# uzh-rpg/EvDeblurNeRF

Hardware: AMD Instinct MI355X
Metric: rays/sec (4096x128 samples, 8x256 MLP) (higher is better)
Workload: dtype f16c (compensated f16: one f16 MFMA product + two block-scaled fp6 MFMA products of the operands' rounding residuals; f32 accumulate; ~2^-15 operands); 1 GPU; nerf8x256 render: 4096 rays x 128 samples per GPU, PE(10,4)+MLP+composite, ndc, viewdirs; rays_per_gpu=4096, samples=128, precision=f16c

## Files before the change

evdeblurnerf_amd/csrc/evd_api.hip:

```cpp
#include <atomic>
#include "evd_common.h"
#include "nerf_mlp.h"
#include "nerf_mlp_kernel.h"
#include "nerf_net.h"
#include "nerf_train.h"
#include "pack.h"

#include <cmath>
#include <cstdint>
#include <cstdlib>
#include <cstring>
#include <vector>

namespace evd {

char* err_buf() {
    static thread_local char buf[512] = {0};
    return buf;
}

int fail(int code, const char* fmt, ...) {
    va_list ap;
    va_start(ap, fmt);
    vsnprintf(err_buf(), 512, fmt, ap);
    va_end(ap);
    return code;
}

int nerf_mlp_generic_dispatch(int prec, int W, const MlpParams& p, hipStream_t st);
int nerf_mlp_pipe_dispatch(int prec, const MlpParams& p, hipStream_t st);
int nerf_mlp_c_dispatch(int W, int D, int skip, const MlpParams& p, hipStream_t st);
int nerf_mlp_c_chunks(int W, int D, int skip, bool train);

static __global__ void k_fold_feature(const float* __restrict__ views_w, const float* __restrict__ views_b, const float* __restrict__ feature_w,
                                      const float* __restrict__ feature_b, int W, int ICV, float* __restrict__ wfold, float* __restrict__ bfold) {
    const int in = W + ICV, rows = W / 2;
    const long i = (long)blockIdx.x * 256 + threadIdx.x;
    if (i < (long)rows * in) {
        const int r = (int)(i / in), c = (int)(i % in);
        if (c >= W) { wfold[i] = views_w[i]; return; }
        double acc = 0.0;
        for (int k = 0; k < W; ++k) acc = fma((double)views_w[(long)r * in + k], (double)feature_w[(long)k * W + c], acc);
        wfold[i] = (float)acc;
    } else if (i < (long)rows * in + rows) {
        const int r = (int)(i - (long)rows * in);
        double acc = 0.0;
        for (int k = 0; k < W; ++k) acc = fma((double)views_w[(long)r * in + k], (double)feature_b[k], acc);
        bfold[r] = (float)(acc + (double)views_b[r]);
    }
}

static int nerf_fold_pack(evd_nerf* n, const float* params, hipStream_t st) {
    if (!n->pipe_cf.data.p) return EVD_OK;
    const int W = n->W, D = n->D, ICV = 3 * (1 + 2 * n->multires_views);
    const long total = n->param_off[n->nparam_blocks], nw = (long)(W / 2) * (W + ICV), nel = nw + W / 2;
    float* ext = (float*)n->fold_arena.p;
    EVD_HIP(hipMemcpyAsync(ext, params, (size_t)total * sizeof(float), hipMemcpyDeviceToDevice, st));
    hipLaunchKernelGGL(k_fold_feature, dim3((unsigned)cdiv(nel, 256L)), dim3(256), 0, st, ext + n->param_off[2 * D], ext + n->param_off[2 * D + 1],
                       ext + n->param_off[2 * D + 2], ext + n->param_off[2 * D + 3], W, ICV, ext + total, ext + total + nw);
    EVD_LAUNCH_CHECK();
    int rc = repack_stream_c(n->pipe_cf, ext, st);
    if (rc) return rc;
    const long nb = (long)(n->bias_f.bytes / sizeof(float));
    hipLaunchKernelGGL(k_gather_f32, dim3((unsigned)cdiv(nb, 256L)), dim3(256), 0, st, (const float*)ext, (const int*)n->bias_f_src.p, nb, (float*)n->bias_f.p);
    EVD_LAUNCH_CHECK();
    return EVD_OK;
}

static std::atomic<long> g_side_spins{0};
static __global__ void k_test_spin(long long ticks) {
    const long long t0 = wall_clock64();
    while (wall_clock64() - t0 < ticks) __builtin_amdgcn_s_sleep(32);
}
int test_side_spin(hipStream_t side) {
    static const int us = [] { const char* e = getenv("EVD_TEST_SIDE_SPIN_US"); return e ? atoi(e) : 0; }();
    if (us <= 0) return EVD_OK;
    hipLaunchKernelGGL(k_test_spin, dim3(1), dim3(64), 0, side, (long long)us * 100);
    EVD_LAUNCH_CHECK();
    g_side_spins.fetch_add(1, std::memory_order_relaxed);
    return EVD_OK;
}
bool test_skip_side_join() {
    static const bool skip = [] { const char* e = getenv("EVD_TEST_SKIP_SIDE_JOIN"); return e && e[0] == '1'; }();
    return skip;
}

}

using namespace evd;

extern "C" {

const char* evd_last_error(void) { return evd::err_buf(); }
long evd_debug_side_spin_count(void) { return evd::g_side_spins.load(std::memory_order_relaxed); }
int evd_version(void) { return 120; }

int evd_device_count(void) {
    int n = 0;
    if (hipGetDeviceCount(&n) != hipSuccess) return fail(EVD_E_NODEVICE, "hipGetDeviceCount failed");
    return n;
}

static int upload_stream(evd_nerf::Packed& dst, const StreamBuilder& sb) { return dst.upload(sb); }

static void nerf_param_sizes(int D, int W, int skip, int L, int Lv, long* sz) {
    const int IC = 3 * (1 + 2 * L), ICV = 3 * (1 + 2 * Lv);
    for (int l = 0; l < D; ++l) {
        sz[2 * l] = (long)W * (l == 0 ? IC : (l - 1 == skip ? W + IC : W));
        sz[2 * l + 1] = W;
    }
    long* h = sz + 2 * D;
    h[0] = (long)(W / 2) * (W + ICV); h[1] = W / 2;
    h[2] = (long)W * W; h[3] = W;
    h[4] = W; h[5] = 1;
    h[6] = 3L * (W / 2); h[7] = 3;
}

int evd_nerf_create(const evd_nerf_desc* d, evd_nerf** out) {
    EVD_REQUIRE(d && out, "evd_nerf_create: null argument");
    EVD_REQUIRE(d->multires >= 0 && d->multires <= PE_L_MAX && d->multires_views >= 0 && pe_ksteps(d->multires_views) <= 4,
                "evd_nerf_create: multires %d / multires_views %d out of range (0..%d / 0..10)", d->multires, d->multires_views, PE_L_MAX);
    const int L = d->multires, Lv = d->multires_views, VKS = pe_ksteps(Lv) <= 2 ? 2 : 4;
    const bool standard = L == PE_L && Lv == PE_LV;
    EVD_REQUIRE(d->W == 256 || d->W == 64, "evd_nerf_create: netwidth %d not built (64, 256)", d->W);
    EVD_REQUIRE(d->D >= 1 && d->D <= EVD_MAX_LAYERS, "evd_nerf_create: netdepth %d out of range", d->D);
    const bool no_views = !d->views_w && !d->feature_w && !d->alpha_w && !d->rgb_w && d->output_w;
    EVD_REQUIRE(no_views || (d->views_w && d->feature_w && d->alpha_w && d->rgb_w),
                "evd_nerf_create: give either the view branch (views / feature / alpha / rgb) or output_linear (use_viewdirs=False)");
    EVD_REQUIRE(!no_views || (d->output_b && (d->output_ch == 4 || d->output_ch == 5)), "evd_nerf_create: output_linear needs its bias and output_ch 4 or 5");
    const int W = d->W, T = W / 32, KS = W / 16, IC = 3 * (1 + 2 * L), ICV = 3 * (1 + 2 * Lv), D = d->D;
    evd_nerf* n = new evd_nerf();
    n->multires = L; n->multires_views = Lv;
    n->D = D; n->W = W; n->skip = d->skip; n->rgb_act = d->rgb_act; n->sigma_act = d->sigma_act; n->rmnear = d->rmnear;
    n->no_views = no_views ? 1 : 0;

    long sz[2 * EVD_MAX_LAYERS + 8];
    nerf_param_sizes(D, W, d->skip, L, Lv, sz);
    n->nparam_blocks = 2 * D + 8;
    if (no_views) {
        sz[2 * D] = (long)d->output_ch * W; sz[2 * D + 1] = d->output_ch;
        n->nparam_blocks = 2 * D + 2;
    }
    long total = 0;
    for (int i = 0; i < n->nparam_blocks; ++i) { n->param_off[i] = total; total += sz[i]; }
    n->param_off[n->nparam_blocks] = total;
    std::vector<float> arena((size_t)total, 0.f);
    {
        const float* srcs[2 * EVD_MAX_LAYERS + 8];
        for (int l = 0; l < D; ++l) { srcs[2 * l] = d->pts_w[l]; srcs[2 * l + 1] = d->pts_b[l]; }
        const float* heads[8] = {d->views_w, d->views_b, d->feature_w, d->feature_b, d->alpha_w, d->alpha_b, d->rgb_w, d->rgb_b};
        for (int i = 0; i < 8; ++i) srcs[2 * D + i] = heads[i];
        if (no_views) { srcs[2 * D] = d->output_w; srcs[2 * D + 1] = d->output_b; }
        for (int i = 0; i < n->nparam_blocks; ++i)
            if (srcs[i]) memcpy(arena.data() + n->param_off[i], srcs[i], sz[i] * sizeof(float));
    }
    const float* A = arena.data();
    auto P = [&](int i) { return A + n->param_off[i]; };
    auto pts_w = [&](int l) { return P(2 * l); };
    const float *views_w = P(2 * D), *feature_w = no_views ? nullptr : P(2 * D + 2), *alpha_w = no_views ? nullptr : P(2 * D + 4), *rgb_w = no_views ? nullptr : P(2 * D + 6);
    const float* output_w = P(2 * D);
    const int out_rows = d->output_ch < 4 ? d->output_ch : 4;

    auto pe_col = [L](int j, int kk) { return pe_src_col(L, 8 * j + (kk & 7), kk >> 3); };
    auto hid_col = [](int j, int kk) { return 16 * j + phi(kk); };
    auto views_col = [&](int j, int kk) {
        if (j < KS) return hid_col(j, kk);
        const int c = pe_src_col(Lv, 8 * (j - KS) + (kk & 7), kk >> 3);
        return c < 0 ? -1 : W + c;
    };
    auto build = [&](StreamBuilder& sb, int pdh) {
        sb.layer(pts_w(0), W, IC, T, PE_KS, true, pe_col);
        for (int l = 1; l < D; ++l) {
            if (l - 1 == d->skip) {
                auto wide_col = [&](int j, int kk) {
                    if (pdh < 0) return j < PE_KS ? pe_col(j, kk) : IC + hid_col(j - PE_KS, kk);
                    if (j < pdh) return IC + hid_col(j, kk);
                    if (j < pdh + PE_KS) return pe_col(j - pdh, kk);
                    return IC + hid_col(j - PE_KS, kk);
                };
                sb.layer(pts_w(l), W, W + IC, T, PE_KS + KS, true, wide_col);
            } else {
                sb.layer(pts_w(l), W, W, T, KS, true, hid_col);
            }
        }
        if (no_views) {
            sb.layer(output_w, out_rows, W, 1, KS, true, hid_col);
            return;
        }
        sb.layer(alpha_w, 1, W, 1, KS, false, hid_col);
        sb.layer(feature_w, W, W, T, KS, false, hid_col);
        sb.layer(views_w, W / 2, W + ICV, T / 2, KS + VKS, false, views_col);
        sb.layer(rgb_w, 3, W / 2, 1, KS / 2, true, hid_col);
    };
    int rc = EVD_OK;
    for (int prec = 0; prec < EVD_NUM_PREC && !rc; ++prec) {
        if (prec == EVD_PREC_F16C) {
            n->nchunks[prec] = n->pipe_chunks[prec] = 0;
            if (no_views || !standard || !nerf_mlp_c_chunks(W, D, d->skip, false)) continue;
            auto build_c = [&](StreamBuilderC& sc, const float* base, bool fold) {
                auto Pb = [&](int i) { return base + n->param_off[i]; };
                sc.arena = base;
                const int KB = KS / 4;
                sc.layer(Pb(0), W, IC, T, PE_KS, 2, pe_col);
                for (int l = 1; l < D; ++l) {
                    if (l - 1 == d->skip) {
                        auto wide_col = [&](int j, int kk) {
                            if (j < 4 * (KB - 1)) return IC + c_hid_col(j, kk);
                            if (j < 4 * (KB - 1) + PE_KS) return pe_col(j - 4 * (KB - 1), kk);
                            return IC + c_hid_col(j - PE_KS, kk);
                        };
                        sc.layer(Pb(2 * l), W, W + IC, T, PE_KS + KS, 2, wide_col);
                    } else {
                        sc.layer(Pb(2 * l), W, W, T, KS, 2, c_hid_col);
                    }
                }
                sc.layer(Pb(2 * D + 4), 1, W, 1, KS, 1, c_hid_col);
                if (!fold) sc.layer(Pb(2 * D + 2), W, W, T, KS, 2, c_hid_col);
                sc.layer(fold ? base + total : Pb(2 * D), W / 2, W + ICV, T / 2, KS + PEV_KS, 2, [&](int j, int kk) {
                    if (j < KS) return c_hid_col(j, kk);
                    const int c = pe_src_col(Lv, 8 * (j - KS) + (kk & 7), kk >> 3);
                    return c < 0 ? -1 : W + c;
                });
                sc.layer(Pb(2 * D + 6), 3, W / 2, 1, KS / 2, 1, c_hid_col);
            };
            StreamBuilderC sc(PIPE_CB);
            build_c(sc, A, false);
            n->pipe_chunks[prec] = (int)(sc.bytes.size() / PIPE_CB);
            if (n->pipe_chunks[prec] != nerf_mlp_c_chunks(W, D, d->skip, true)) rc = fail(EVD_E_INVALID, "evd_nerf_create: f16c stream has %d chunks, kernel expects %d", n->pipe_chunks[prec], nerf_mlp_c_chunks(W, D, d->skip, true));
            if (!rc) rc = n->pipe_c.upload(sc);
            if (rc) continue;
            const long nfold = (long)(W / 2) * (W + ICV) + W / 2;
            std::vector<float> ext((size_t)(total + nfold), 0.f);
            StreamBuilderC sf(PIPE_CB);
            build_c(sf, ext.data(), true);
            n->fold_chunks = (int)(sf.bytes.size() / PIPE_CB);
            if (n->fold_chunks != nerf_mlp_c_chunks(W, D, d->skip, false)) rc = fail(EVD_E_INVALID, "evd_nerf_create: folded f16c stream has %d chunks, kernel expects %d", n->fold_chunks, nerf_mlp_c_chunks(W, D, d->skip, false));
            if (!rc) rc = n->pipe_cf.upload(sf);
            if (!rc) rc = n->fold_arena.alloc(ext.size() * sizeof(float));
            continue;
        }
        StreamBuilder sb(prec);
        sb.arena = A;
        build(sb, -1);
        n->nchunks[prec] = (int)(sb.bytes.size() / chunk_bytes(prec));
        rc = upload_stream(n->stream[prec], sb);
        n->pipe_chunks[prec] = 0;
        if (!rc && !no_views && standard && nerf_pipe_built(prec, W, D, d->skip)) {
            StreamBuilder sp(prec, PIPE_CB);
            sp.arena = A;
            sp.group = nerf_group(prec);
            build(sp, KS - 2 * nerf_group(prec));
            n->pipe_chunks[prec] = (int)(sp.bytes.size() / PIPE_CB);
            rc = upload_stream(n->pipe[prec], sp);
        }
        if (rc || !is_train_prec(prec) || !n->pipe_chunks[prec]) continue;
        auto put = [&](int which, auto fill) {
            StreamBuilder sb2(prec, PIPE_CB);
            sb2.arena = A;
            sb2.group = 1;
            fill(sb2);
            return upload_stream(n->bwd[prec][which], sb2);
        };
        rc = put(EVD_BWD_RGB, [&](StreamBuilder& b) { b.layer_transposed(rgb_w, 3, W / 2, 0, W / 2, nullptr, 0, T / 2, 1, true, [](int, int kk) { return kk < 3 ? kk : -1; }); });
        if (!rc) rc = put(EVD_BWD_VIEWS, [&](StreamBuilder& b) { b.layer_transposed(views_w, W / 2, W + ICV, 0, W, nullptr, 0, T, KS / 2, true, hid_col); });
        if (!rc) rc = put(EVD_BWD_HEAD, [&](StreamBuilder& b) {
            b.layer_transposed(feature_w, W, W, 0, W, alpha_w, 1, T, KS + 1, true, [&](int j, int kk) { return j < KS ? hid_col(j, kk) : (kk == 0 ? W : -1); });
        });
        auto enc_row = [](int L_, int idx) { const int j = idx / 16, kk = phi_inv(idx % 16); return pe_src_col(L_, 8 * j + (kk & 7), kk >> 3); };
        auto enc_layer = [&](StreamBuilder& b, const float* Wm, int in_dim, int col0, int L_, int tiles, int ksteps) {
            b.layer_at(tiles, ksteps, true, [&](int t, int r) { const int c = enc_row(L_, 32 * t + r); return c < 0 ? -1 : col0 + c; }, hid_col,
                       [=](int r, int c) { return Wm + (size_t)c * in_dim + r; });
        };
        if (!rc) rc = put(EVD_BWD_PE0, [&](StreamBuilder& b) { enc_layer(b, pts_w(0), IC, 0, PE_L, 2, KS); });
        if (!rc && d->skip >= 0 && d->skip + 1 < D) rc = put(EVD_BWD_PESKIP, [&](StreamBuilder& b) { enc_layer(b, pts_w(d->skip + 1), W + IC, 0, PE_L, 2, KS); });
        if (!rc) rc = put(EVD_BWD_DIR, [&](StreamBuilder& b) { enc_layer(b, views_w, W + ICV, W, PE_LV, 1, KS / 2); });
        for (int l = 1; l < D && !rc; ++l) {
            const bool wide = l - 1 == d->skip;
            rc = put(EVD_BWD_HIDDEN1 + l - 1, [&](StreamBuilder& b) { b.layer_transposed(pts_w(l), W, wide ? W + IC : W, wide ? IC : 0, W, nullptr, 0, T, KS, true, hid_col); });
        }
    }
    if (rc) { evd_nerf_destroy(n); return rc; }
    {
        std::vector<int> m(MAP_TOTAL, -1);
        for (int i = 0; i < 256; ++i) {
            m[MAP_HID + i] = hid_col(i / 16, i % 16);
            m[MAP_HID_SKIP + i] = IC + hid_col(i / 16, i % 16);
        }
        for (int i = 0; i < 64; ++i) m[MAP_PE + i] = pe_col(i / 16, i % 16);
        for (int i = 0; i < 32; ++i) {
            const int c = pe_src_col(Lv, 8 * (i / 16) + (i % 16 & 7), (i % 16) >> 3);
            m[MAP_DIR + i] = c < 0 ? -1 : W + c;
        }
        for (int i = 0; i < 3; ++i) m[MAP_RGB + i] = i;
        m[MAP_ALPHA] = 0;
        if ((rc = n->wmaps.upload(m.data(), m.size() * sizeof(int)))) { evd_nerf_destroy(n); return rc; }
    }
    std::vector<float> b;
    std::vector<int32_t> bsrc;
    auto push = [&](int block, int out_dim, int tiles) {
        for (int i = 0; i < tiles * 32; ++i) {
            b.push_back(i < out_dim ? P(block)[i] : 0.f);
            bsrc.push_back(i < out_dim ? (int32_t)(n->param_off[block] + i) : -1);
        }
    };
    for (int l = 0; l < D; ++l) push(2 * l + 1, W, T);
    if (no_views) {
        push(2 * D + 1, out_rows, 1);
    } else {
        push(2 * D + 5, 1, 1);
        push(2 * D + 3, W, T);
        push(2 * D + 1, W / 2, T / 2);
        push(2 * D + 7, 3, 1);
    }
    rc = n->bias.upload(b.data(), b.size() * sizeof(float));
    if (!rc) rc = n->bias_src.upload(bsrc.data(), bsrc.size() * sizeof(int32_t));
    if (!rc && n->pipe_cf.data.p) {
        const long nw = (long)(W / 2) * (W + ICV);
        std::vector<int32_t> fsrc(bsrc.begin(), bsrc.begin() + (D * T + 1) * 32);
        for (int i = 0; i < (T / 2) * 32; ++i) fsrc.push_back((int32_t)(total + nw + i));
        fsrc.insert(fsrc.end(), bsrc.end() - 32, bsrc.end());
        rc = n->bias_f_src.upload(fsrc.data(), fsrc.size() * sizeof(int32_t));
        if (!rc) rc = n->bias_f.alloc(fsrc.size() * sizeof(float));
        DevBuf dev_params;
        if (!rc) rc = dev_params.upload(arena.data(), arena.size() * sizeof(float));
        if (!rc) rc = nerf_fold_pack(n, (const float*)dev_params.p, nullptr);
        if (!rc && hipStreamSynchronize(nullptr) != hipSuccess) rc = fail(EVD_E_HIP, "evd_nerf_create: the folded f16c stream could not be packed");
        dev_params.release();
    }
    if (rc) { evd_nerf_destroy(n); return rc; }
    *out = n;
    return EVD_OK;
}

void evd_nerf_destroy(evd_nerf* n) {
    if (!n) return;
    for (int i = 0; i < EVD_NUM_PREC; ++i) {
        n->stream[i].release();
        n->pipe[i].release();
        for (int k = 0; k < EVD_BWD_NSTREAMS; ++k) n->bwd[i][k].release();
    }
    n->wmaps.release();
    n->batch.release();
    n->bias.release();
    n->bias_src.release();
    n->pipe_c.release();
    n->pipe_cf.release();
    n->bias_f.release();
    n->bias_f_src.release();
    n->fold_arena.release();
    n->side.release();
    delete n;
}

long evd_nerf_param_count(const evd_nerf* net) { return net ? net->param_off[net->nparam_blocks] : 0; }

int evd_nerf_param_blocks(const evd_nerf* net, long* offsets, int capacity) {
    EVD_REQUIRE(net, "evd_nerf_param_blocks: null network");
    if (offsets)
        for (int i = 0; i <= net->nparam_blocks && i < capacity; ++i) offsets[i] = net->param_off[i];
    return net->nparam_blocks;
}

int evd_nerf_load_params(evd_nerf* net, const float* params, void* stream) {
    EVD_REQUIRE(net && params, "evd_nerf_load_params: null argument");
    hipStream_t st = as_stream(stream);
    int rc;
    std::vector<PackedStream*> all;
    for (int i = 0; i < EVD_NUM_PREC; ++i) {
        all.push_back(&net->stream[i]);
        all.push_back(&net->pipe[i]);
        for (int k = 0; k < EVD_BWD_NSTREAMS; ++k) all.push_back(&net->bwd[i][k]);
    }
    if ((rc = repack_batch(net->batch, all, params, st))) return rc;
    if ((rc = repack_stream_c(net->pipe_c, params, st))) return rc;
    const long nb = (long)(net->bias.bytes / sizeof(float));
    hipLaunchKernelGGL(k_gather_f32, dim3((unsigned)cdiv(nb, 256L)), dim3(256), 0, st, params, (const int*)net->bias_src.p, nb, (float*)net->bias.p);
    EVD_LAUNCH_CHECK();
    return nerf_fold_pack(net, params, st);
}

size_t evd_nerf_stream_bytes(const evd_nerf* net, int precision) {
    if (!net || precision < 0 || precision >= EVD_NUM_PREC) return 0;
    if (precision == EVD_PREC_F16C) return net->pipe_cf.data.bytes;
    return net->pipe_chunks[precision] ? net->pipe[precision].data.bytes : net->stream[precision].data.bytes;
}

int evd_nerf_mlp(const evd_nerf* net, int precision, const float* ray_batch, const float* z, long R, int S,
                 float* raw, float* feature, int feature_kind, void* stream) {
    EVD_REQUIRE(net && ray_batch && z && raw, "evd_nerf_mlp: null argument");
    EVD_REQUIRE(precision >= 0 && precision < EVD_NUM_PREC, "evd_nerf_mlp: unknown precision %d", precision);
    EVD_REQUIRE(R >= 0 && S >= 1, "evd_nerf_mlp: bad shape R=%ld S=%d", R, S);
    EVD_REQUIRE(!feature || feature_kind == 1 || feature_kind == 2, "evd_nerf_mlp: feature_kind must be 1 or 2");
    if (R == 0) return EVD_OK;
    MlpParams p{};
    const bool piped = net->pipe_chunks[precision] > 0;
    p.wstream = (const char*)(piped ? net->pipe[precision].data.p : net->stream[precision].data.p);
    p.bias = (const float*)net->bias.p;
    p.ray_batch = ray_batch; p.z = z; p.nsamp = R * (long)S; p.S = S; p.ncol = net->no_views ? 8 : 11; p.no_views = net->no_views;
    p.pe_l = net->multires; p.pe_lv = net->multires_views;
    EVD_REQUIRE(!(net->no_views && feature && feature_kind == 1), "evd_nerf_mlp: a use_viewdirs=False network has no after_linear feature (nerf.py:159)");
    EVD_REQUIRE(!net->no_views || precision != EVD_PREC_F16C, "evd_nerf_mlp: EVD_PREC_F16C is not built for use_viewdirs=False networks");
    p.D = net->D; p.skip = net->skip; p.nchunks = piped ? net->pipe_chunks[precision] : net->nchunks[precision]; p.nbias = (int)(net->bias.bytes / sizeof(float));
    p.raw = raw; p.feature = feature; p.feature_kind = feature ? feature_kind : 0; p.act = nullptr; p.wscale = nullptr;
    if (precision == EVD_PREC_F16C) {
        EVD_REQUIRE(net->pipe_chunks[precision] > 0, "evd_nerf_mlp: EVD_PREC_F16C is built for netdepth 8, netwidth 256, skips [4], multires 10 / 4 only");
        EVD_REQUIRE(!feature, "evd_nerf_mlp: EVD_PREC_F16C has no feature-row variant (use EVD_PREC_F16X3)");
        p.wstream = (const char*)net->pipe_cf.data.p;
        p.nchunks = net->fold_chunks;
        p.wscale = (const unsigned*)net->pipe_cf.scales.p;
        p.bias = (const float*)net->bias_f.p;
        p.nbias = (int)(net->bias_f.bytes / sizeof(float));
        return nerf_mlp_c_dispatch(net->W, net->D, net->skip, p, as_stream(stream));
    }
    if (piped) return nerf_mlp_pipe_dispatch(precision, p, as_stream(stream));
    return nerf_mlp_generic_dispatch(precision, net->W, p, as_stream(stream));
}

static size_t align256(size_t x) { return (x + 255) & ~(size_t)255; }

size_t evd_nerf_render_workspace_bytes(const evd_render_cfg* cfg, long R) {
    if (!cfg || R < 0) return 0;
    const size_t S = cfg->N_samples, Ni = cfg->N_importance > 0 ? cfg->N_importance : 0, St = S + Ni, r = (size_t)R;
    size_t b = 0;
    b += align256(r * 11 * 4);
    b += align256(r * St * 4);
    b += align256(r * S * 4);
    b += align256(r * St * 16);
    b += align256(r * St * 4);
    b += align256(r * S * 4);
    b += align256(r * (Ni ? Ni : 1) * 4);
    return b + 256;
}

}
static float* render_z_slot(const evd_render_cfg* cfg, long R, const evd_render_out* out, void* workspace) {
    const int S = cfg->N_samples, Ni = cfg->N_importance > 0 ? cfg->N_importance : 0, St = S + Ni;
    char* w = (char*)(((uintptr_t)workspace + 255) & ~(uintptr_t)255);
    w += align256((size_t)R * 11 * 4) + align256((size_t)R * St * 4);
    float* z0 = (float*)w;
    return Ni ? (out->z_vals0 ? out->z_vals0 : z0) : (out->z_vals ? out->z_vals : z0);
}
static int render_rays_impl(const evd_nerf* coarse, const evd_nerf* fine, const evd_render_cfg* cfg, const float* rb,
                            long R, const float* t_rand, const float* u, const float* noise0, const float* noise1,
                            evd_render_out* out, void* workspace, size_t workspace_bytes, void* stream, bool z_done) {
    EVD_REQUIRE(coarse && cfg && out && (rb || R == 0), "evd_nerf_render_rays: null argument");
    EVD_REQUIRE((cfg->use_viewdirs != 0) == (coarse->no_views == 0) && (!fine || fine->no_views == coarse->no_views),
                "evd_nerf_render_rays: cfg->use_viewdirs does not match the networks (view branch vs output_linear)");
    const int nc = cfg->use_viewdirs ? 11 : 8;
    EVD_REQUIRE(cfg->N_samples >= 1, "evd_nerf_render_rays: N_samples must be >= 1");
    EVD_REQUIRE(cfg->N_importance <= 0 || fine, "evd_nerf_render_rays: N_importance > 0 needs the fine network");
    EVD_REQUIRE(cfg->N_importance <= 0 || cfg->N_samples >= 3, "evd_nerf_render_rays: hierarchical sampling needs N_samples >= 3");
    EVD_REQUIRE(!(cfg->perturb > 0.f) || (t_rand && (cfg->N_importance <= 0 || u)),
                "evd_nerf_render_rays: perturb > 0 needs explicit t_rand (and u) draws");
    if (R == 0) return EVD_OK;
    const size_t need = evd_nerf_render_workspace_bytes(cfg, R);
    if (!workspace || workspace_bytes < need)
        return fail(EVD_E_WORKSPACE, "evd_nerf_render_rays: workspace %zu < %zu bytes", workspace_bytes, need);
    const int S = cfg->N_samples, Ni = cfg->N_importance > 0 ? cfg->N_importance : 0, St = S + Ni;
    char* w = (char*)(((uintptr_t)workspace + 255) & ~(uintptr_t)255);
    auto take = [&](size_t bytes) { char* p = w; w += align256(bytes); return (float*)p; };
    const size_t r = (size_t)R;
    (void)take(r * 11 * 4);
    float* z2 = take(r * St * 4);
    float* z0 = take(r * S * 4);
    float* raw = take(r * St * 16);
    float* wts = take(r * St * 4);
    float* wts0 = take(r * S * 4);
    float* zs = take(r * (Ni ? Ni : 1) * 4);
    int rc;
    float* zc = (Ni ? (out->z_vals0 ? out->z_vals0 : z0) : (out->z_vals ? out->z_vals : z0));
    if (!z_done && (rc = evd_sample_z(cfg, rb, nc, R, t_rand, zc, stream))) return rc;
    auto pass = [&](const evd_nerf* net, const float* z, int Sp, const float* noise, float* rgb, float* depth, float* acc,
                    float* weights, float* raw_out, float* feat) -> int {
        int rc2 = evd_nerf_mlp(net, cfg->precision, rb, z, R, Sp, raw_out, feat, out->feature_kind ? out->feature_kind : 1, stream);
        if (rc2) return rc2;
        const float thr = (!cfg->is_train && net->rmnear > 0.f) ? (float)((double)net->rmnear / 128.0) : 0.f;
        return evd_raw2outputs(raw_out, z, rb + 3, nc, R, Sp, 4, 3, 0, 3, net->rgb_act, net->sigma_act, cfg->white_bkgd, thr,
                               noise, rgb, nullptr, acc, weights, depth, nullptr, 0, nullptr, stream);
    };
    if (!Ni) {
        float* wo = out->weights ? out->weights : wts;
        float* ro = out->raw ? out->raw : raw;
        return pass(coarse, zc, S, noise0, out->rgb, out->depth, out->acc, wo, ro, out->feature);
    }
    float* w0 = out->weights0 ? out->weights0 : wts0;
    if ((rc = pass(coarse, zc, S, noise0, out->rgb0, out->depth0, out->acc0, w0, raw, nullptr))) return rc;
    float* zm = out->z_vals ? out->z_vals : z2;
    if ((rc = evd_sample_pdf_merge(zc, w0, R, S, Ni, cfg->perturb == 0.f, u, zs, zm, nullptr, out->z_std, stream))) return rc;
    float* wo = out->weights ? out->weights : wts;
    float* ro = out->raw ? out->raw : raw;
    return pass(fine, zm, St, noise1, out->rgb, out->depth, out->acc, wo, ro, out->feature);
}

extern "C" {
// ... 23 lines not shown
```

evdeblurnerf_amd/csrc/kernel_nerf_mlp_pipe_f16c.hip:

```cpp
#include "nerf_mlp_c_kernel.h"

namespace evd {

int nerf_mlp_c_chunks(int W, int D, int skip, bool train) {
    if (!nerf_c_built(W, D, skip)) return 0;
    return train ? nerf_c_chunks<256, 8, 4, true>() : nerf_c_chunks<256, 8, 4, false>();
}

int nerf_mlp_c_dispatch(int W, int D, int skip, const MlpParams& p, hipStream_t st) {
    if (nerf_c_built(W, D, skip)) return launch_nerf_c<256, 8, 4>(p, st);
    return fail(EVD_E_INVALID, "evd_nerf_mlp: EVD_PREC_F16C is built for netdepth 8, netwidth 256, skips [4] only");
}

}
```

evdeblurnerf_amd/csrc/nerf_mlp.h:

```cpp
#pragma once

#include <cstddef>
#include <cstdint>

namespace evd {

constexpr int PE_L = 10;
constexpr int PE_LV = 4;
constexpr int PE_KS = (3 * PE_L + 2 + 7) / 8;
constexpr int PEV_KS = (3 * PE_LV + 2 + 7) / 8;
constexpr int PE_L_MAX = (8 * PE_KS - 2) / 3;
__host__ __device__ constexpr int pe_ksteps(int L) { return (3 * L + 2 + 7) / 8; }

__host__ __device__ constexpr int phi(int kk) { return 8 * ((kk & 7) >> 2) + 4 * (kk >> 3) + (kk & 3); }
__host__ __device__ constexpr int phi_inv(int p) { return (p & 3) | ((p >> 3) << 2) | (((p >> 2) & 1) << 3); }

__host__ __device__ constexpr int pe_src_col(int L, int q, int h) {
    return q < 3 * L ? 3 + 6 * (q / 3) + 3 * h + (q % 3) : (q == 3 * L ? h : (q == 3 * L + 1 ? (h == 0 ? 2 : -1) : -1));
}

constexpr bool is_half_prec(int prec) { return prec == 2  || prec == 3 ; }
constexpr bool is_train_prec(int prec) { return is_half_prec(prec) || prec == 1 ; }
constexpr int frag_bytes(int prec) { return is_half_prec(prec) ? 1024 : 2048; }
constexpr int mlp_threads(int prec) { return is_half_prec(prec) ? 512 : 256; }
constexpr int chunk_bytes(int prec) { return mlp_threads(prec) * 64; }
constexpr int frags_per_chunk(int prec) { return chunk_bytes(prec) / frag_bytes(prec); }

constexpr int nerf_group(int prec) { return 1; }

struct MlpParams {
    const char* wstream;
    const float* bias;
    const float* ray_batch;
    const float* z;
    long nsamp;
    int S, ncol, D, skip, nchunks, nbias;
    float* raw;
    float* feature;
    int feature_kind;
    char* act;
    int pe_l, pe_lv;
    int no_views;
    const unsigned* wscale;
};

namespace astore {
constexpr int PE = 0, DIR = 4, H0 = 6;
constexpr int F = H0 + 16 * 8, HV = F + 16, FWD_END = HV + 8;
constexpr int G_RGB = FWD_END, G_ALPHA = G_RGB + 1;
constexpr int D_HV = G_ALPHA + 1, D_F = D_HV + 8, D_H0 = D_F + 16;
constexpr int D_PE0 = D_H0 + 16 * 8, D_PE5 = D_PE0 + PE_KS, D_DIRG = D_PE5 + PE_KS;
constexpr int M_H0 = D_DIRG + PEV_KS, M_HV = M_H0 + 8;
constexpr int TILE_FRAGS = M_HV + 1;
constexpr long TILE_BYTES = (long)TILE_FRAGS * 1024;
constexpr long tile_bytes(int prec) { return (long)TILE_FRAGS * frag_bytes(prec); }
}

}
```

evdeblurnerf_amd/csrc/nerf_mlp_c_kernel.h:

```cpp
#pragma once

#include "mlp_pipe_c.h"

namespace evd {

template <int W, int D, int SKIP, bool TRAIN = false> struct NerfNetC {
    static constexpr int T = W / 32, KB = W / 64;
    static constexpr bool FOLD = !TRAIN;
    static constexpr int slot(int s) { return TRAIN ? s : -1; }
    static constexpr int oslot(int l) { return slot(astore::H0 + 16 * l); }
    static constexpr int pslot(int l) { return slot(astore::H0 + 16 * l + 4 * (KB - 1)); }
    static constexpr int mslot(int l) { return slot(astore::M_H0 + l); }
    static_assert(!TRAIN || (W == 256 && D == 8), "the activation store is laid out for the 8 x 256 network");
    static_assert(PE_KS == 4 && PEV_KS == 2 && T % 2 == 0 && KB >= 2, "block structure of the encodings and the hidden width");
    static constexpr bool is_wide(int l) { return l - 1 == SKIP; }
    typedef CLayer<1, 4, T, 2, true, false, 0, 0, 0, false, 0, 2, oslot(0), -1, mslot(0)> L0;
    static constexpr int CH_HID = CLayer<KB, 4, T, 2, true, false, 0, 0, 2, true, KB - 1, 2>::NCHUNKS;
    static constexpr int CH_WIDE = CLayer<KB + 1, 4, T, 2, true, false, 0, 0, 2, true, KB, 2>::NCHUNKS;
    static constexpr int chunk0(int l) {
        int c = L0::NCHUNKS;
        for (int i = 1; i < l; ++i) c += is_wide(i) ? CH_WIDE : CH_HID;
        return c;
    }
    static constexpr int PARH = L0::PAR_OUT;
    static_assert((T / 2) % 2 == 0, "accumulator parity");
    template <int l> using Hidden = std::conditional_t<is_wide(l),
        CLayer<KB + 1, 4, T, 2, true, false, chunk0(l), PARH, 2, true, KB, l == D - 1 ? 1 : 2, oslot(l), pslot(l - 1), mslot(l), mslot(l - 1), 4 * (KB - 1)>,
        CLayer<KB, 4, T, 2, true, false, chunk0(l), PARH, 2, true, KB - 1, l == D - 1 ? 1 : 2, oslot(l), pslot(l - 1), mslot(l), mslot(l - 1)>>;
    typedef CLayer<KB, 4, 1, 1, false, true, chunk0(D), PARH, 2, true, KB - 1, 2, -1, pslot(D - 1), -1, mslot(D - 1)> Alpha;
    typedef CLayer<KB, 4, T, 2, false, false, Alpha::CHUNK0 + Alpha::NCHUNKS, Alpha::PAR_OUT, 0, false, 0, 2, slot(astore::F)> Feature;
    typedef std::conditional_t<FOLD,
        CLayer<KB + 1, 2, T / 2, 2, true, false, Alpha::CHUNK0 + Alpha::NCHUNKS, Alpha::PAR_OUT, 0, false, 0, 1>,
        CLayer<KB + 1, 2, T / 2, 2, true, false, Feature::CHUNK0 + Feature::NCHUNKS, Feature::PAR_OUT, 2, false, KB - 1, 1, slot(astore::HV),
               slot(astore::F + 4 * (KB - 1)), slot(astore::M_HV)>> Views;
    typedef CLayer<KB / 2, 4, 1, 1, false, true, Views::CHUNK0 + Views::NCHUNKS, Views::PAR_OUT, 2, true, KB / 2 - 1, 0, -1, slot(astore::HV + 4 * (KB / 2 - 1)), -1,
                   slot(astore::M_HV)> Rgb;
    static constexpr int NCH = Rgb::CHUNK0 + Rgb::NCHUNKS;
    static constexpr int NTILES = D * T + 1 + (FOLD ? 0 : T) + T / 2 + 1;
    static_assert(D >= 2 && NTILES * 32 <= CCfg::BIAS_WORDS / 2, "bias / row-scale block");
};

template <class N, class ST> struct NerfCtxC {
    ST st;
    CPipe pp;
    XBlk buf[2][N::KB];
    XBlk pe, pev;
    lds_f32_p bias;
    int lane;
    CAct act;
};

template <class N, class ST, int l, int D, bool TRAIN = false> struct HiddenLoopC {
    static __device__ __forceinline__ void run(NerfCtxC<N, ST>& cx) {
        typedef typename N::template Hidden<l> L;
        constexpr int KB = N::KB, T = N::T;
        lds_f32_p lb = cx.bias + l * T * 32;
        if constexpr (l + 1 < D) {
            typedef typename N::template Hidden<l + 1> NX;
            step<L, NX>(cx, lb);
            HiddenLoopC<N, ST, l + 1, D, TRAIN>::run(cx);
        } else {
            step<L, typename N::Alpha>(cx, lb);
        }
    }
    template <class L, class NX> static __device__ __forceinline__ void step(NerfCtxC<N, ST>& cx, lds_f32_p lb) {
        constexpr int KB = N::KB;
        if constexpr (N::is_wide(l)) {
            XBlk wide[KB + 1];
#pragma unroll
            for (int j = 0; j < KB - 1; ++j) wide[j] = cx.buf[(l - 1) & 1][j];
            wide[KB - 1] = cx.pe;
            c_layer<L, NX, ST, KB + 1, KB, TRAIN>(cx.st, cx.pp, wide, cx.buf[l & 1], nullptr, lb, cx.lane, cx.act);
        } else {
            c_layer<L, NX, ST, KB, KB, TRAIN>(cx.st, cx.pp, cx.buf[(l - 1) & 1], cx.buf[l & 1], nullptr, lb, cx.lane, cx.act);
        }
    }
};

template <int W, int D, int SKIP, bool TRAIN = false>
__global__ __launch_bounds__(CCfg::NT, 1) void k_nerf_mlp_c(const MlpParams p) {
    typedef NerfNetC<W, D, SKIP, TRAIN> N;
    typedef CStream<N::NCH> ST;
    constexpr int T = N::T, KB = N::KB;
    extern __shared__ __attribute__((aligned(16))) char smem[];

    pipe_fp16_saturate<EVD_PREC_F16>();
    const int tid = threadIdx.x, lane = tid & 63, wave = tid >> 6;
    const int n = lane & 31, h = lane >> 5;
    ST st0;
    st0.start_issue(p.wstream, smem, tid);
    float* bias = reinterpret_cast<float*>(smem + CCfg::RING);
    {
        constexpr int NB = (CCfg::BIAS_WORDS / 2 / 4 + CCfg::NT - 1) / CCfg::NT;
        f32x4 bv[NB];
        u32x4 sv[NB];
#pragma unroll
        for (int q = 0; q < NB; ++q) {
            const int i = (tid + q * CCfg::NT) * 4;
            bv[q] = i < p.nbias ? *reinterpret_cast<const f32x4*>(p.bias + i) : f32x4{0.f, 0.f, 0.f, 0.f};
            sv[q] = i < p.nbias ? *reinterpret_cast<const u32x4*>(p.wscale + i) : u32x4{0u, 0u, 0u, 0u};
        }
#pragma unroll
        for (int q = 0; q < NB; ++q) {
            const int i = (tid + q * CCfg::NT) * 4;
            if (i < p.nbias) {
                *reinterpret_cast<f32x4*>(bias + i) = bv[q];
                *reinterpret_cast<u32x4*>(reinterpret_cast<unsigned*>(bias) + CCfg::BIAS_WORDS / 2 + i) = sv[q];
            }
        }
    }
    unsigned bias_off = lds_offset_of(bias);
    asm volatile("" : "+v"(bias_off));
    const lds_f32_p lbias = (lds_f32_p)(unsigned long)bias_off;

    const long ntile = TRAIN ? (p.nsamp + 255) / 256 * (256 / CCfg::SAMPLES) : (p.nsamp + CCfg::SAMPLES - 1) / CCfg::SAMPLES;
    for (long tile = blockIdx.x;;) {
    NerfCtxC<N, ST> cx;
    cx.st = st0;
    cx.bias = lbias;
    cx.lane = lane;
    const long smp = tile * CCfg::SAMPLES + wave * 32 + n;
    const bool valid = smp < p.nsamp;
    const long sidx = valid ? smp : p.nsamp - 1;
    {
        const long ray = sidx / p.S;
        const float* rb = p.ray_batch + ray * p.ncol;
        const float zv = p.z[sidx];
        float pts[3], vd[3];
#pragma unroll
        for (int c = 0; c < 3; ++c) {
            pts[c] = __fadd_rn(rb[c], __fmul_rn(rb[3 + c], zv));
            vd[c] = rb[8 + c];
        }
        c_encode<PE_L, PE_KS>(pts, h, cx.pe);
        c_encode<PE_LV, PEV_KS>(vd, h, cx.pev);
    }
    cx.act = CAct{};
    if constexpr (TRAIN) {
        const long t32 = __builtin_amdgcn_readfirstlane((int)(tile * (CCfg::SAMPLES / 32) + wave));
        cx.act.base = p.act + t32 * astore::TILE_BYTES;
        cx.act.voff = lane * 16;
        c_store_input<PE_KS>(cx.act, astore::PE, cx.pe);
        c_store_input<PEV_KS>(cx.act, astore::DIR, cx.pev);
    }

    cx.st.start_wait();
    c_prime<typename N::L0>(cx.st, cx.pp, lbias, lane);
    {
        XBlk in_pe[1];
        in_pe[0] = cx.pe;
        c_layer<typename N::L0, typename N::template Hidden<1>, ST, 1, KB, TRAIN>(cx.st, cx.pp, in_pe, cx.buf[0], nullptr, lbias, lane, cx.act);
    }
    HiddenLoopC<N, ST, 1, D, TRAIN>::run(cx);

    XBlk (&hact)[KB] = cx.buf[(D - 1) & 1];
    lds_f32_p lb = lbias + D * T * 32;
    float araw[4], rraw[4];
    XBlk none[1];
    typedef std::conditional_t<N::FOLD, typename N::Views, typename N::Feature> AfterAlpha;
    c_layer<typename N::Alpha, AfterAlpha, ST, KB, 1, TRAIN>(cx.st, cx.pp, hact, none, araw, lb, lane, cx.act);
    lb += 32;
    XBlk hbuf[KB / 2];
    if constexpr (N::FOLD) {
        XBlk hv[KB + 1];
#pragma unroll
        for (int j = 0; j < KB; ++j) hv[j] = hact[j];
        hv[KB] = cx.pev;
        c_layer<typename N::Views, typename N::Rgb, ST, KB + 1, KB / 2, TRAIN>(cx.st, cx.pp, hv, hbuf, nullptr, lb, lane, cx.act);
    } else {
        XBlk vin[KB + 1];
        c_layer<typename N::Feature, typename N::Views, ST, KB, KB + 1, TRAIN>(cx.st, cx.pp, hact, vin, nullptr, lb, lane, cx.act);
        lb += T * 32;
        vin[KB] = cx.pev;
        c_layer<typename N::Views, typename N::Rgb, ST, KB + 1, KB / 2, TRAIN>(cx.st, cx.pp, vin, hbuf, nullptr, lb, lane, cx.act);
    }
    lb += (T / 2) * 32;
    c_layer<typename N::Rgb, void, ST, KB / 2, 1, TRAIN>(cx.st, cx.pp, hbuf, none, rraw, lb, lane, cx.act);
    const bool more = tile + gridDim.x < ntile;
    if (more) cx.st.restart_issue();

    if (h == 0 && valid) {
        f32x4 o = {rraw[0], rraw[1], rraw[2], araw[0]};
        *reinterpret_cast<f32x4*>(p.raw + sidx * 4) = o;
    }
    if (!more) break;
    tile += gridDim.x;
    }
}

template <int W, int D, int SKIP, bool TRAIN = false> constexpr int nerf_c_chunks() { return NerfNetC<W, D, SKIP, TRAIN>::NCH; }

template <int W, int D, int SKIP, bool TRAIN = false>
static int launch_nerf_c(const MlpParams& p, hipStream_t st) {
    typedef NerfNetC<W, D, SKIP, TRAIN> N;
    const long tiles = TRAIN ? cdiv(p.nsamp, 256L) * (256 / CCfg::SAMPLES) : cdiv(p.nsamp, CCfg::SAMPLES);
    const long blocks = cmin_l(tiles, (long)c_persistent_blocks());
    const size_t lds = CCfg::TOTAL;
    EVD_SET_MAX_LDS((&k_nerf_mlp_c<W, D, SKIP, TRAIN>), lds);
    if (TRAIN != (p.act != nullptr)) return fail(EVD_E_INVALID, "evd_nerf_mlp (f16c): the activation store goes with the training launch");
    if (p.nbias != N::NTILES * 32) return fail(EVD_E_INVALID, "evd_nerf_mlp (f16c): %d bias floats, kernel expects %d", p.nbias, N::NTILES * 32);
    if (p.nchunks != N::NCH) return fail(EVD_E_INVALID, "evd_nerf_mlp (f16c): packed stream has %d chunks, kernel expects %d", p.nchunks, N::NCH);
    if (!p.wscale) return fail(EVD_E_INVALID, "evd_nerf_mlp (f16c): no row scales");
    hipLaunchKernelGGL((k_nerf_mlp_c<W, D, SKIP, TRAIN>), dim3((unsigned)blocks), dim3(CCfg::NT), lds, st, p);
    EVD_LAUNCH_CHECK();
    return EVD_OK;
}

constexpr bool nerf_c_built(int W, int D, int skip) { return W == 256 && D == 8 && skip == 4; }


}
```

evdeblurnerf_amd/csrc/nerf_net.h:

```cpp
#pragma once

#include "evd_common.h"
#include "pack.h"

enum { EVD_BWD_RGB = 0, EVD_BWD_VIEWS, EVD_BWD_HEAD, EVD_BWD_PE0, EVD_BWD_PESKIP, EVD_BWD_DIR, EVD_BWD_HIDDEN1, EVD_BWD_NSTREAMS = EVD_BWD_HIDDEN1 + EVD_MAX_LAYERS };

struct evd_nerf {
    typedef evd::PackedStream Packed;
    int D, W, skip, rgb_act, sigma_act;
    int multires = 10, multires_views = 4;
    int no_views = 0;
    float rmnear;
    Packed stream[EVD_NUM_PREC];
    int nchunks[EVD_NUM_PREC];
    Packed pipe[EVD_NUM_PREC];
    int pipe_chunks[EVD_NUM_PREC];
    evd::DevBuf bias, bias_src;
    evd::PackedStreamC pipe_c;
    evd::PackedStreamC pipe_cf;
    evd::DevBuf bias_f, bias_f_src, fold_arena;
    int fold_chunks = 0;
    Packed bwd[EVD_NUM_PREC][EVD_BWD_NSTREAMS];
    evd::DevBuf wmaps;
    int nparam_blocks;
    long param_off[2 * EVD_MAX_LAYERS + 9];
    evd::RepackBatch batch;
    mutable evd::SideStream side;
};
```

Baseline: 5.606 million rays/s.

## Hoist view-direction encoding out of per-sample MFMA into per-ray bias rows

Adds a ray-aligned variant of the folded f16c inference kernel, used when samples per ray are a multiple of 32. Since every sample in a 32-row tile shares one view direction, the view-direction positional-encoding columns are dropped from the Views layer's MFMA K dimension. Instead their contribution is computed once per ray in f32 with scalar FMAs from an LDS copy of the direction weights, and added into a per-wave bias row. This removes one K block of compensated MFMA work per sample. In exchange it adds extra LDS, a per-tile lane-broadcast dot product, and a separate repacked weight stream plus direction-weight buffer.

```diff
diff --git a/evdeblurnerf_amd/csrc/evd_api.hip b/evdeblurnerf_amd/csrc/evd_api.hip
--- a/evdeblurnerf_amd/csrc/evd_api.hip
+++ b/evdeblurnerf_amd/csrc/evd_api.hip
@@ -31,14 +31,20 @@
 int nerf_mlp_pipe_dispatch(int prec, const MlpParams& p, hipStream_t st);
 int nerf_mlp_c_dispatch(int W, int D, int skip, const MlpParams& p, hipStream_t st);
 int nerf_mlp_c_chunks(int W, int D, int skip, bool train);
+int nerf_mlp_c_ray_chunks(int W, int D, int skip);
 
 static __global__ void k_fold_feature(const float* __restrict__ views_w, const float* __restrict__ views_b, const float* __restrict__ feature_w,
-                                      const float* __restrict__ feature_b, int W, int ICV, float* __restrict__ wfold, float* __restrict__ bfold) {
+                                      const float* __restrict__ feature_b, int W, int ICV, float* __restrict__ wfold, float* __restrict__ bfold,
+                                      float* __restrict__ dirw) {
     const int in = W + ICV, rows = W / 2;
     const long i = (long)blockIdx.x * 256 + threadIdx.x;
     if (i < (long)rows * in) {
         const int r = (int)(i / in), c = (int)(i % in);
-        if (c >= W) { wfold[i] = views_w[i]; return; }
+        if (c >= W) {
+            wfold[i] = views_w[i];
+            if (dirw) dirw[r * NERF_DIRW_STRIDE + (c - W)] = views_w[i];
+            return;
+        }
         double acc = 0.0;
         for (int k = 0; k < W; ++k) acc = fma((double)views_w[(long)r * in + k], (double)feature_w[(long)k * W + c], acc);
         wfold[i] = (float)acc;
@@ -57,9 +63,10 @@
     float* ext = (float*)n->fold_arena.p;
     EVD_HIP(hipMemcpyAsync(ext, params, (size_t)total * sizeof(float), hipMemcpyDeviceToDevice, st));
     hipLaunchKernelGGL(k_fold_feature, dim3((unsigned)cdiv(nel, 256L)), dim3(256), 0, st, ext + n->param_off[2 * D], ext + n->param_off[2 * D + 1],
-                       ext + n->param_off[2 * D + 2], ext + n->param_off[2 * D + 3], W, ICV, ext + total, ext + total + nw);
+                       ext + n->param_off[2 * D + 2], ext + n->param_off[2 * D + 3], W, ICV, ext + total, ext + total + nw, (float*)n->dir_w.p);
     EVD_LAUNCH_CHECK();
     int rc = repack_stream_c(n->pipe_cf, ext, st);
+    if (!rc) rc = repack_stream_c(n->pipe_cr, ext, st);
     if (rc) return rc;
     const long nb = (long)(n->bias_f.bytes / sizeof(float));
     hipLaunchKernelGGL(k_gather_f32, dim3((unsigned)cdiv(nb, 256L)), dim3(256), 0, st, (const float*)ext, (const int*)n->bias_f_src.p, nb, (float*)n->bias_f.p);
@@ -197,7 +204,7 @@
         if (prec == EVD_PREC_F16C) {
             n->nchunks[prec] = n->pipe_chunks[prec] = 0;
             if (no_views || !standard || !nerf_mlp_c_chunks(W, D, d->skip, false)) continue;
-            auto build_c = [&](StreamBuilderC& sc, const float* base, bool fold) {
+            auto build_c = [&](StreamBuilderC& sc, const float* base, bool fold, bool dir) {
                 auto Pb = [&](int i) { return base + n->param_off[i]; };
                 sc.arena = base;
                 const int KB = KS / 4;
@@ -216,7 +223,7 @@
                 }
                 sc.layer(Pb(2 * D + 4), 1, W, 1, KS, 1, c_hid_col);
                 if (!fold) sc.layer(Pb(2 * D + 2), W, W, T, KS, 2, c_hid_col);
-                sc.layer(fold ? base + total : Pb(2 * D), W / 2, W + ICV, T / 2, KS + PEV_KS, 2, [&](int j, int kk) {
+                sc.layer(fold ? base + total : Pb(2 * D), W / 2, W + ICV, T / 2, dir ? KS + PEV_KS : KS, 2, [&](int j, int kk) {
                     if (j < KS) return c_hid_col(j, kk);
                     const int c = pe_src_col(Lv, 8 * (j - KS) + (kk & 7), kk >> 3);
                     return c < 0 ? -1 : W + c;
@@ -224,7 +231,7 @@
                 sc.layer(Pb(2 * D + 6), 3, W / 2, 1, KS / 2, 1, c_hid_col);
             };
             StreamBuilderC sc(PIPE_CB);
-            build_c(sc, A, false);
+            build_c(sc, A, false, true);
             n->pipe_chunks[prec] = (int)(sc.bytes.size() / PIPE_CB);
             if (n->pipe_chunks[prec] != nerf_mlp_c_chunks(W, D, d->skip, true)) rc = fail(EVD_E_INVALID, "evd_nerf_create: f16c stream has %d chunks, kernel expects %d", n->pipe_chunks[prec], nerf_mlp_c_chunks(W, D, d->skip, true));
             if (!rc) rc = n->pipe_c.upload(sc);
@@ -232,11 +239,20 @@
             const long nfold = (long)(W / 2) * (W + ICV) + W / 2;
             std::vector<float> ext((size_t)(total + nfold), 0.f);
             StreamBuilderC sf(PIPE_CB);
-            build_c(sf, ext.data(), true);
+            build_c(sf, ext.data(), true, true);
             n->fold_chunks = (int)(sf.bytes.size() / PIPE_CB);
             if (n->fold_chunks != nerf_mlp_c_chunks(W, D, d->skip, false)) rc = fail(EVD_E_INVALID, "evd_nerf_create: folded f16c stream has %d chunks, kernel expects %d", n->fold_chunks, nerf_mlp_c_chunks(W, D, d->skip, false));
             if (!rc) rc = n->pipe_cf.upload(sf);
             if (!rc) rc = n->fold_arena.alloc(ext.size() * sizeof(float));
+            if (rc) continue;
+            StreamBuilderC sr(PIPE_CB);
+            build_c(sr, ext.data(), true, false);
+            n->ray_chunks = (int)(sr.bytes.size() / PIPE_CB);
+            if (n->ray_chunks != nerf_mlp_c_ray_chunks(W, D, d->skip)) rc = fail(EVD_E_INVALID, "evd_nerf_create: ray-aligned f16c stream has %d chunks, kernel expects %d", n->ray_chunks, nerf_mlp_c_ray_chunks(W, D, d->skip));
+            if (!rc) rc = n->pipe_cr.upload(sr);
+            static_assert(NERF_DIRW_STRIDE >= 3 * (1 + 2 * PE_LV), "direction columns");
+            const std::vector<float> dz((size_t)(W / 2) * NERF_DIRW_STRIDE, 0.f);
+            if (!rc) rc = n->dir_w.upload(dz.data(), dz.size() * sizeof(float));
             continue;
         }
         StreamBuilder sb(prec);
@@ -345,6 +361,8 @@
     n->bias_src.release();
     n->pipe_c.release();
     n->pipe_cf.release();
+    n->pipe_cr.release();
+    n->dir_w.release();
     n->bias_f.release();
     n->bias_f_src.release();
     n->fold_arena.release();
@@ -410,6 +428,12 @@
         p.wscale = (const unsigned*)net->pipe_cf.scales.p;
         p.bias = (const float*)net->bias_f.p;
         p.nbias = (int)(net->bias_f.bytes / sizeof(float));
+        if (S % 32 == 0) {
+            p.wstream = (const char*)net->pipe_cr.data.p;
+            p.nchunks = net->ray_chunks;
+            p.wscale = (const unsigned*)net->pipe_cr.scales.p;
+            p.dirw = (const float*)net->dir_w.p;
+        }
         return nerf_mlp_c_dispatch(net->W, net->D, net->skip, p, as_stream(stream));
     }
     if (piped) return nerf_mlp_pipe_dispatch(precision, p, as_stream(stream));
diff --git a/evdeblurnerf_amd/csrc/kernel_nerf_mlp_pipe_f16c.hip b/evdeblurnerf_amd/csrc/kernel_nerf_mlp_pipe_f16c.hip
--- a/evdeblurnerf_amd/csrc/kernel_nerf_mlp_pipe_f16c.hip
+++ b/evdeblurnerf_amd/csrc/kernel_nerf_mlp_pipe_f16c.hip
@@ -6,10 +6,11 @@
     if (!nerf_c_built(W, D, skip)) return 0;
     return train ? nerf_c_chunks<256, 8, 4, true>() : nerf_c_chunks<256, 8, 4, false>();
 }
+int nerf_mlp_c_ray_chunks(int W, int D, int skip) { return nerf_c_built(W, D, skip) ? nerf_c_chunks<256, 8, 4, false, true>() : 0; }
 
 int nerf_mlp_c_dispatch(int W, int D, int skip, const MlpParams& p, hipStream_t st) {
-    if (nerf_c_built(W, D, skip)) return launch_nerf_c<256, 8, 4>(p, st);
-    return fail(EVD_E_INVALID, "evd_nerf_mlp: EVD_PREC_F16C is built for netdepth 8, netwidth 256, skips [4] only");
+    if (!nerf_c_built(W, D, skip)) return fail(EVD_E_INVALID, "evd_nerf_mlp: EVD_PREC_F16C is built for netdepth 8, netwidth 256, skips [4] only");
+    return p.dirw ? launch_nerf_c<256, 8, 4, false, true>(p, st) : launch_nerf_c<256, 8, 4>(p, st);
 }
 
 }
diff --git a/evdeblurnerf_amd/csrc/nerf_mlp.h b/evdeblurnerf_amd/csrc/nerf_mlp.h
--- a/evdeblurnerf_amd/csrc/nerf_mlp.h
+++ b/evdeblurnerf_amd/csrc/nerf_mlp.h
@@ -28,6 +28,8 @@
 
 constexpr int nerf_group(int prec) { return 1; }
 
+constexpr int NERF_DIRW_STRIDE = 28;
+
 struct MlpParams {
     const char* wstream;
     const float* bias;
@@ -42,6 +44,7 @@
     int pe_l, pe_lv;
     int no_views;
     const unsigned* wscale;
+    const float* dirw;
 };
 
 namespace astore {
diff --git a/evdeblurnerf_amd/csrc/nerf_mlp_c_kernel.h b/evdeblurnerf_amd/csrc/nerf_mlp_c_kernel.h
--- a/evdeblurnerf_amd/csrc/nerf_mlp_c_kernel.h
+++ b/evdeblurnerf_amd/csrc/nerf_mlp_c_kernel.h
@@ -4,9 +4,11 @@
 
 namespace evd {
 
-template <int W, int D, int SKIP, bool TRAIN = false> struct NerfNetC {
+template <int W, int D, int SKIP, bool TRAIN = false, bool RAY_ = false> struct NerfNetC {
     static constexpr int T = W / 32, KB = W / 64;
     static constexpr bool FOLD = !TRAIN;
+    static constexpr bool RAY = RAY_;
+    static_assert(!RAY_ || FOLD, "the ray-aligned variant is the folded inference kernel's");
     static constexpr int slot(int s) { return TRAIN ? s : -1; }
     static constexpr int oslot(int l) { return slot(astore::H0 + 16 * l); }
     static constexpr int pslot(int l) { return slot(astore::H0 + 16 * l + 4 * (KB - 1)); }
@@ -30,7 +32,8 @@
     typedef CLayer<KB, 4, 1, 1, false, true, chunk0(D), PARH, 2, true, KB - 1, 2, -1, pslot(D - 1), -1, mslot(D - 1)> Alpha;
     typedef CLayer<KB, 4, T, 2, false, false, Alpha::CHUNK0 + Alpha::NCHUNKS, Alpha::PAR_OUT, 0, false, 0, 2, slot(astore::F)> Feature;
     typedef std::conditional_t<FOLD,
-        CLayer<KB + 1, 2, T / 2, 2, true, false, Alpha::CHUNK0 + Alpha::NCHUNKS, Alpha::PAR_OUT, 0, false, 0, 1>,
+        std::conditional_t<RAY, CLayer<KB, 4, T / 2, 2, true, false, Alpha::CHUNK0 + Alpha::NCHUNKS, Alpha::PAR_OUT, 0, false, 0, 1>,
+                           CLayer<KB + 1, 2, T / 2, 2, true, false, Alpha::CHUNK0 + Alpha::NCHUNKS, Alpha::PAR_OUT, 0, false, 0, 1>>,
         CLayer<KB + 1, 2, T / 2, 2, true, false, Feature::CHUNK0 + Feature::NCHUNKS, Feature::PAR_OUT, 2, false, KB - 1, 1, slot(astore::HV),
                slot(astore::F + 4 * (KB - 1)), slot(astore::M_HV)>> Views;
     typedef CLayer<KB / 2, 4, 1, 1, false, true, Views::CHUNK0 + Views::NCHUNKS, Views::PAR_OUT, 2, true, KB / 2 - 1, 0, -1, slot(astore::HV + 4 * (KB / 2 - 1)), -1,
@@ -38,6 +41,16 @@
     static constexpr int NCH = Rgb::CHUNK0 + Rgb::NCHUNKS;
     static constexpr int NTILES = D * T + 1 + (FOLD ? 0 : T) + T / 2 + 1;
     static_assert(D >= 2 && NTILES * 32 <= CCfg::BIAS_WORDS / 2, "bias / row-scale block");
+    static constexpr int HEAD0 = D * T * 32;
+};
+
+template <class N> struct RayDir {
+    static constexpr int ICV = 3 * (1 + 2 * PE_LV), DWS = NERF_DIRW_STRIDE, ROWS_V = (N::T / 2) * 32, ROWS = (1 + N::T / 2 + 1) * 32;
+    static constexpr int SC_OFF = CCfg::BIAS_WORDS / 2;
+    static constexpr int DIRW = SC_OFF + CCfg::NW * ROWS, WORDS = DIRW + ROWS_V * DWS;
+    static constexpr int LDS = N::RAY ? CCfg::TOTAL + WORDS * 4 : CCfg::TOTAL;
+    static_assert(CCfg::NW * ROWS <= SC_OFF && ROWS_V == 128 && DWS % 4 == 0 && (DWS / 4) % 2 == 1 && DWS >= ICV && ICV <= 64 && LDS <= 160 * 1024,
+                  "ray-aligned LDS block");
 };
 
 template <class N, class ST> struct NerfCtxC {
@@ -77,9 +90,10 @@
     }
 };
 
-template <int W, int D, int SKIP, bool TRAIN = false>
+template <int W, int D, int SKIP, bool TRAIN = false, bool RAY = false>
 __global__ __launch_bounds__(CCfg::NT, 1) void k_nerf_mlp_c(const MlpParams p) {
-    typedef NerfNetC<W, D, SKIP, TRAIN> N;
+    typedef NerfNetC<W, D, SKIP, TRAIN, RAY> N;
+    typedef RayDir<N> RD;
     typedef CStream<N::NCH> ST;
     constexpr int T = N::T, KB = N::KB;
     extern __shared__ __attribute__((aligned(16))) char smem[];
@@ -90,6 +104,22 @@
     ST st0;
     st0.start_issue(p.wstream, smem, tid);
     float* bias = reinterpret_cast<float*>(smem + CCfg::RING);
+    constexpr int NQ = (RD::ROWS_V * RD::DWS / 4 + CCfg::NT - 1) / CCfg::NT;
+    f32x4 wv[NQ];
+    float hb[RD::ROWS / 64];
+    unsigned hs[RD::ROWS / 64];
+    if constexpr (RAY) {
+#pragma unroll
+        for (int q = 0; q < NQ; ++q) {
+            const int i = tid + q * CCfg::NT;
+            wv[q] = i < RD::ROWS_V * RD::DWS / 4 ? reinterpret_cast<const f32x4*>(p.dirw)[i] : f32x4{0.f, 0.f, 0.f, 0.f};
+        }
+#pragma unroll
+        for (int q = 0; q < RD::ROWS / 64; ++q) {
+            hb[q] = p.bias[N::HEAD0 + lane + 64 * q];
+            hs[q] = p.wscale[N::HEAD0 + lane + 64 * q];
+        }
+    }
     {
         constexpr int NB = (CCfg::BIAS_WORDS / 2 / 4 + CCfg::NT - 1) / CCfg::NT;
         f32x4 bv[NB];
@@ -112,6 +142,27 @@
     unsigned bias_off = lds_offset_of(bias);
     asm volatile("" : "+v"(bias_off));
     const lds_f32_p lbias = (lds_f32_p)(unsigned long)bias_off;
+    float* const rrows = reinterpret_cast<float*>(smem + CCfg::TOTAL) + wave * RD::ROWS;
+    const f32x4* const dirw = reinterpret_cast<const f32x4*>(smem + CCfg::TOTAL + RD::DIRW * 4);
+    lds_f32_p lrows = lbias;
+    if constexpr (RAY) {
+#pragma unroll
+        for (int q = 0; q < NQ; ++q) {
+            const int i = tid + q * CCfg::NT;
+            if (i < RD::ROWS_V * RD::DWS / 4) reinterpret_cast<f32x4*>(smem + CCfg::TOTAL + RD::DIRW * 4)[i] = wv[q];
+        }
+#pragma unroll
+        for (int q = 0; q < RD::ROWS / 64; ++q) {
+            rrows[lane + 64 * q] = hb[q];
+            reinterpret_cast<unsigned*>(rrows)[RD::SC_OFF + lane + 64 * q] = hs[q];
+        }
+        unsigned rows_off = lds_offset_of(rrows);
+        asm volatile("" : "+v"(rows_off));
+        lrows = (lds_f32_p)(unsigned long)rows_off;
+        __syncthreads();
+    }
+    const int pe_i = lane < RD::ICV ? lane : 0, pe_c = pe_i % 3;
+    const float pe_scale = (float)(1 << (pe_i < 3 ? 0 : (pe_i - 3) / 6)), pe_phase = (pe_i >= 3 && ((pe_i - 3) / 3) % 2) ? 0.25f : 0.f;
 
     const long ntile = TRAIN ? (p.nsamp + 255) / 256 * (256 / CCfg::SAMPLES) : (p.nsamp + CCfg::SAMPLES - 1) / CCfg::SAMPLES;
     for (long tile = blockIdx.x;;) {
@@ -133,7 +184,30 @@
             vd[c] = rb[8 + c];
         }
         c_encode<PE_L, PE_KS>(pts, h, cx.pe);
-        c_encode<PE_LV, PEV_KS>(vd, h, cx.pev);
+        if constexpr (!RAY) {
+            c_encode<PE_LV, PEV_KS>(vd, h, cx.pev);
+        } else {
+            f32x4 w0[RD::DWS / 4], w1[RD::DWS / 4];
+#pragma unroll
+            for (int j = 0; j < RD::DWS / 4; ++j) {
+                w0[j] = dirw[lane * (RD::DWS / 4) + j];
+                w1[j] = dirw[(lane + 64) * (RD::DWS / 4) + j];
+            }
+            const float x = pe_c == 0 ? vd[0] : (pe_c == 1 ? vd[1] : vd[2]);
+            const float thi = x * 0.15915494309189535f;
+            const float tlo = fmaf(x, 0.15915494309189535f, -thi) + x * 6.4206383e-09f;
+            const float sv = __builtin_amdgcn_sinf(fmaf(tlo, pe_scale, __builtin_amdgcn_fractf(thi * pe_scale) + pe_phase));
+            const int ev = __builtin_bit_cast(int, lane < 3 ? x : sv);
+            float t0 = 0.f, t1 = 0.f;
+#pragma unroll
+            for (int k = 0; k < RD::ICV; ++k) {
+                const float e = __builtin_bit_cast(float, __builtin_amdgcn_readlane(ev, k));
+                t0 = fmaf(w0[k / 4][k % 4], e, t0);
+                t1 = fmaf(w1[k / 4][k % 4], e, t1);
+            }
+            rrows[32 + lane] = t0 + bias[N::HEAD0 + 32 + lane];
+            rrows[32 + 64 + lane] = t1 + bias[N::HEAD0 + 32 + 64 + lane];
+        }
     }
     cx.act = CAct{};
     if constexpr (TRAIN) {
@@ -154,14 +228,16 @@
     HiddenLoopC<N, ST, 1, D, TRAIN>::run(cx);
 
     XBlk (&hact)[KB] = cx.buf[(D - 1) & 1];
-    lds_f32_p lb = lbias + D * T * 32;
+    lds_f32_p lb = RAY ? lrows : lbias + N::HEAD0;
     float araw[4], rraw[4];
     XBlk none[1];
     typedef std::conditional_t<N::FOLD, typename N::Views, typename N::Feature> AfterAlpha;
     c_layer<typename N::Alpha, AfterAlpha, ST, KB, 1, TRAIN>(cx.st, cx.pp, hact, none, araw, lb, lane, cx.act);
     lb += 32;
     XBlk hbuf[KB / 2];
-    if constexpr (N::FOLD) {
+    if constexpr (RAY) {
+        c_layer<typename N::Views, typename N::Rgb, ST, KB, KB / 2, TRAIN>(cx.st, cx.pp, hact, hbuf, nullptr, lb, lane, cx.act);
+    } else if constexpr (N::FOLD) {
         XBlk hv[KB + 1];
 #pragma unroll
         for (int j = 0; j < KB; ++j) hv[j] = hact[j];
@@ -188,20 +264,22 @@
     }
 }
 
-template <int W, int D, int SKIP, bool TRAIN = false> constexpr int nerf_c_chunks() { return NerfNetC<W, D, SKIP, TRAIN>::NCH; }
-
-template <int W, int D, int SKIP, bool TRAIN = false>
+template <int W, int D, int SKIP, bool TRAIN = false, bool RAY = false> constexpr int nerf_c_chunks() { return NerfNetC<W, D, SKIP, TRAIN, RAY>::NCH; }
+
+template <int W, int D, int SKIP, bool TRAIN = false, bool RAY = false>
 static int launch_nerf_c(const MlpParams& p, hipStream_t st) {
-    typedef NerfNetC<W, D, SKIP, TRAIN> N;
+    typedef NerfNetC<W, D, SKIP, TRAIN, RAY> N;
     const long tiles = TRAIN ? cdiv(p.nsamp, 256L) * (256 / CCfg::SAMPLES) : cdiv(p.nsamp, CCfg::SAMPLES);
     const long blocks = cmin_l(tiles, (long)c_persistent_blocks());
-    const size_t lds = CCfg::TOTAL;
-    EVD_SET_MAX_LDS((&k_nerf_mlp_c<W, D, SKIP, TRAIN>), lds);
+    const size_t lds = RayDir<N>::LDS;
+    EVD_SET_MAX_LDS((&k_nerf_mlp_c<W, D, SKIP, TRAIN, RAY>), lds);
+    if (RAY != (p.dirw != nullptr)) return fail(EVD_E_INVALID, "evd_nerf_mlp (f16c): the direction columns go with the ray-aligned launch");
+    if (RAY && p.S % 32 != 0) return fail(EVD_E_INVALID, "evd_nerf_mlp (f16c): the ray-aligned kernel needs S %% 32 == 0, got %d", p.S);
     if (TRAIN != (p.act != nullptr)) return fail(EVD_E_INVALID, "evd_nerf_mlp (f16c): the activation store goes with the training launch");
     if (p.nbias != N::NTILES * 32) return fail(EVD_E_INVALID, "evd_nerf_mlp (f16c): %d bias floats, kernel expects %d", p.nbias, N::NTILES * 32);
     if (p.nchunks != N::NCH) return fail(EVD_E_INVALID, "evd_nerf_mlp (f16c): packed stream has %d chunks, kernel expects %d", p.nchunks, N::NCH);
     if (!p.wscale) return fail(EVD_E_INVALID, "evd_nerf_mlp (f16c): no row scales");
-    hipLaunchKernelGGL((k_nerf_mlp_c<W, D, SKIP, TRAIN>), dim3((unsigned)blocks), dim3(CCfg::NT), lds, st, p);
+    hipLaunchKernelGGL((k_nerf_mlp_c<W, D, SKIP, TRAIN, RAY>), dim3((unsigned)blocks), dim3(CCfg::NT), lds, st, p);
     EVD_LAUNCH_CHECK();
     return EVD_OK;
 }
diff --git a/evdeblurnerf_amd/csrc/nerf_net.h b/evdeblurnerf_amd/csrc/nerf_net.h
--- a/evdeblurnerf_amd/csrc/nerf_net.h
+++ b/evdeblurnerf_amd/csrc/nerf_net.h
@@ -20,6 +20,9 @@
     evd::PackedStreamC pipe_cf;
     evd::DevBuf bias_f, bias_f_src, fold_arena;
     int fold_chunks = 0;
+    evd::PackedStreamC pipe_cr;
+    evd::DevBuf dir_w;
+    int ray_chunks = 0;
     Packed bwd[EVD_NUM_PREC][EVD_BWD_NSTREAMS];
     evd::DevBuf wmaps;
     int nparam_blocks;
```

New measurement: 5.633 million rays/s, median of 6. No clear change (+0.5%).
